# jy0205/Pyramid-Flow

Hardware: NVIDIA H100
Metric: dit_step_latent_tokens_per_sec (higher is better)
Workload: dtype bf16

## Files before the change

### pyramid_flow_b200/csrc/pf_attn.cu

```cuda
#include <algorithm>
#include <vector>

#include "../../include/pf_b200.h"
#include "pf_common.cuh"

namespace pf {

constexpr int ATT_BM = 128;
constexpr int ATT_BN = 128;
constexpr int ATT_HD = 64;
constexpr int ATT_STAGES = 2;
constexpr int ATT_THREADS = 384;
constexpr int ATT_TILE_BYTES = ATT_BN * ATT_HD * 2;
constexpr int ATT_SMEM_BYTES = (1 + 2 * ATT_STAGES) * ATT_TILE_BYTES + 1024;

struct AttnArgs {
  __nv_bfloat16* out;
  long long ldo;
  int batch, heads, seq, q_tiles;
  float scale_log2;
  const int* seg;
  const int* time;
  const int* sched;
  int sched_stride;
  __nv_bfloat16* peer_out[PF_MAX_PEERS];
  int peer_count, peer_chunk_rows, peer_col_begin;
};

__global__ void __launch_bounds__(ATT_THREADS, 1)
attn_fwd_kernel(const __grid_constant__ CUtensorMap tm_q, const __grid_constant__ CUtensorMap tm_k,
                const __grid_constant__ CUtensorMap tm_v, const AttnArgs a) {
  extern __shared__ uint8_t smem_raw[];
  uint8_t* smem = reinterpret_cast<uint8_t*>((reinterpret_cast<uintptr_t>(smem_raw) + 1023) & ~uintptr_t(1023));
  uint8_t* smem_q = smem;
  uint8_t* smem_k = smem + ATT_TILE_BYTES;
  uint8_t* smem_v = smem_k + ATT_STAGES * ATT_TILE_BYTES;

  __shared__ __align__(8) uint64_t bar_q;
  __shared__ __align__(8) uint64_t k_full[ATT_STAGES], k_empty[ATT_STAGES], v_full[ATT_STAGES], v_empty[ATT_STAGES];

  const int warp = threadIdx.x >> 5;
  const int lane = threadIdx.x & 31;
  const int wgroup = warp >> 2;
  const int qt = a.q_tiles - 1 - static_cast<int>(blockIdx.x);
  const int h = blockIdx.y;
  const int b = blockIdx.z;
  const int bh = b * a.heads + h;
  const int* sched = a.sched + (static_cast<size_t>(b) * a.q_tiles + qt) * a.sched_stride;
  const int n_kv = sched[0];

  if (threadIdx.x == 0) {
    tma_prefetch_desc(&tm_q);
    tma_prefetch_desc(&tm_k);
    tma_prefetch_desc(&tm_v);
    mbar_init(&bar_q, 1);
    for (int i = 0; i < ATT_STAGES; ++i) {
      mbar_init(&k_full[i], 1);
      mbar_init(&k_empty[i], 8);
      mbar_init(&v_full[i], 1);
      mbar_init(&v_empty[i], 8);
    }
    fence_barrier_init();
  }
  __syncthreads();

  if (wgroup == 0) {
    setmaxnreg_dec<40>();
    if (warp == 0 && elect_one()) {
      mbar_arrive_expect_tx(&bar_q, ATT_TILE_BYTES);
      tma_load_3d(smem_q, &tm_q, &bar_q, 0, qt * ATT_BM, bh);
      int st = 0;
      uint32_t ph = 0;
      for (int j = 0; j < n_kv; ++j) {
        const int kt = sched[1 + j] >> 1;
        mbar_wait(&k_empty[st], ph ^ 1);
        mbar_arrive_expect_tx(&k_full[st], ATT_TILE_BYTES);
        tma_load_3d(smem_k + st * ATT_TILE_BYTES, &tm_k, &k_full[st], 0, kt * ATT_BN, bh);
        mbar_wait(&v_empty[st], ph ^ 1);
        mbar_arrive_expect_tx(&v_full[st], ATT_TILE_BYTES);
        tma_load_3d(smem_v + st * ATT_TILE_BYTES, &tm_v, &v_full[st], 0, kt * ATT_BN, bh);
        if (++st == ATT_STAGES) {
          st = 0;
          ph ^= 1;
        }
      }
    }
    return;
  }

  setmaxnreg_inc<232>();
  const int wg = wgroup - 1;
  const int g4 = lane >> 2, t4 = lane & 3;
  const int row0 = wg * 64 + (warp & 3) * 16 + g4;
  const float c = a.scale_log2;
  const int* sg = a.seg + static_cast<size_t>(b) * a.seq;
  const int* tm = a.time + static_cast<size_t>(b) * a.seq;
  int seg_q[2], time_q[2];
#pragma unroll
  for (int r = 0; r < 2; ++r) {
    const int qpos = qt * ATT_BM + row0 + 8 * r;
    const bool q_valid = qpos < a.seq;
    seg_q[r] = q_valid ? sg[qpos] : -0x7fffffff;
    time_q[r] = q_valid ? tm[qpos] : -0x7fffffff;
  }
  float m_run[2] = {-INFINITY, -INFINITY};
  float l_run[2] = {0.f, 0.f};
  float o[32];
#pragma unroll
  for (int i = 0; i < 32; ++i) o[i] = 0.f;

  mbar_wait(&bar_q, 0);
  const uint64_t dq = make_smem_desc_kmajor_sw128(smem_u32(smem_q) + wg * (64 * 128));
  int st = 0;
  uint32_t ph = 0;
  for (int j = 0; j < n_kv; ++j) {
    const int entry = sched[1 + j];
    const int kt = entry >> 1;
    const bool masked = (entry & 1) != 0;

    float s[64];
    mbar_wait(&k_full[st], ph);
    {
      const uint64_t dk = make_smem_desc_kmajor_sw128(smem_u32(smem_k + st * ATT_TILE_BYTES));
      wgmma_fence();
#pragma unroll
      for (int kk = 0; kk < ATT_HD / 16; ++kk) wgmma_ss_n128(s, dq + 2 * kk, dk + 2 * kk, kk != 0 ? 1u : 0u);
      wgmma_commit();
      wgmma_wait<0>();
      wgmma_reg_fence(s);
    }
    if (lane == 0) mbar_arrive(&k_empty[st]);

    if (masked) {
#pragma unroll
      for (int i = 0; i < 16; ++i) {
#pragma unroll
        for (int e = 0; e < 2; ++e) {
          const int kv = kt * ATT_BN + 8 * i + 2 * t4 + e;
          int sk = 0x7fffffff, tk = 0x7fffffff;
          if (kv < a.seq) {
            sk = __ldg(sg + kv);
            tk = __ldg(tm + kv);
          }
          if (!(sk == seg_q[0] && tk <= time_q[0])) s[4 * i + e] = -INFINITY;
          if (!(sk == seg_q[1] && tk <= time_q[1])) s[4 * i + 2 + e] = -INFINITY;
        }
      }
    }

    float alpha[2];
#pragma unroll
    for (int r = 0; r < 2; ++r) {
      float mx = -INFINITY;
#pragma unroll
      for (int i = 0; i < 16; ++i) mx = fmaxf(mx, fmaxf(s[4 * i + 2 * r], s[4 * i + 2 * r + 1]));
      mx = fmaxf(mx, __shfl_xor_sync(0xffffffffu, mx, 1));
      mx = fmaxf(mx, __shfl_xor_sync(0xffffffffu, mx, 2));
      const float m_new = fmaxf(m_run[r], mx);
      alpha[r] = (m_new == -INFINITY) ? 1.f : ex2_approx_f((m_run[r] - m_new) * c);
      m_run[r] = m_new;
      const float m_ref = (m_new == -INFINITY) ? 0.f : m_new * c;
      float sum = 0.f;
#pragma unroll
      for (int i = 0; i < 16; ++i) {
        const float p0 = ex2_approx_f(fmaf(s[4 * i + 2 * r], c, -m_ref));
        const float p1 = ex2_approx_f(fmaf(s[4 * i + 2 * r + 1], c, -m_ref));
        s[4 * i + 2 * r] = p0;
        s[4 * i + 2 * r + 1] = p1;
        sum += p0 + p1;
      }
      l_run[r] = l_run[r] * alpha[r] + sum;
    }
#pragma unroll
    for (int i = 0; i < 8; ++i) {
      o[4 * i + 0] *= alpha[0];
      o[4 * i + 1] *= alpha[0];
      o[4 * i + 2] *= alpha[1];
      o[4 * i + 3] *= alpha[1];
    }

    mbar_wait(&v_full[st], ph);
    {
      const uint32_t sv = smem_u32(smem_v + st * ATT_TILE_BYTES);
      uint32_t pa[ATT_BN / 16][4];
#pragma unroll
      for (int kk = 0; kk < ATT_BN / 16; ++kk) {
        pa[kk][0] = pack_bf16x2(s[8 * kk + 0], s[8 * kk + 1]);
        pa[kk][1] = pack_bf16x2(s[8 * kk + 2], s[8 * kk + 3]);
        pa[kk][2] = pack_bf16x2(s[8 * kk + 4], s[8 * kk + 5]);
        pa[kk][3] = pack_bf16x2(s[8 * kk + 6], s[8 * kk + 7]);
      }
      wgmma_reg_fence(o);
      wgmma_fence();
#pragma unroll
      for (int kk = 0; kk < ATT_BN / 16; ++kk) {
        const uint64_t dv = make_smem_desc(sv + kk * 2048, ATT_BN * 128, 1024);
        wgmma_rs_n64_tb(o, pa[kk], dv);
      }
      wgmma_commit();
      wgmma_wait<0>();
      wgmma_reg_fence(o);
    }
    if (lane == 0) mbar_arrive(&v_empty[st]);
    if (++st == ATT_STAGES) {
      st = 0;
      ph ^= 1;
    }
  }

#pragma unroll
  for (int r = 0; r < 2; ++r) {
    float l = l_run[r];
    l += __shfl_xor_sync(0xffffffffu, l, 1);
    l += __shfl_xor_sync(0xffffffffu, l, 2);
    const float inv = (l > 0.f) ? 1.f / l : 0.f;
    const int qpos = qt * ATT_BM + row0 + 8 * r;
    if (qpos >= a.seq) continue;
    __nv_bfloat16* dst;
    if (a.peer_count > 1) {
      const int pr = qpos / a.peer_chunk_rows;
      dst = a.peer_out[pr] + static_cast<size_t>(qpos - pr * a.peer_chunk_rows) * a.ldo + a.peer_col_begin + h * ATT_HD;
    } else {
      dst = a.out + (static_cast<size_t>(b) * a.seq + qpos) * a.ldo + h * ATT_HD;
    }
#pragma unroll
    for (int i = 0; i < 8; ++i)
      *reinterpret_cast<uint32_t*>(dst + 8 * i + 2 * t4) = pack_bf16x2(o[4 * i + 2 * r] * inv, o[4 * i + 2 * r + 1] * inv);
  }
}

int warmup_attn() {
  return ensure_dyn_smem(reinterpret_cast<const void*>(attn_fwd_kernel), ATT_SMEM_BYTES, "attn_fwd_kernel");
}

}

extern "C" int pf_attn_build_schedule(const int32_t* seg, const int32_t* time, int32_t batch, int32_t seq,
                                      int32_t* out, int64_t* allowed_pairs) {
  using namespace pf;
  PF_REQUIRE(batch > 0 && seq > 0, "pf_attn_build_schedule: bad shape");
  const int tiles = (seq + 127) / 128;
  const int stride = 1 + tiles;
  if (out == nullptr) return stride;
  PF_REQUIRE(seg && time, "pf_attn_build_schedule: null ids");
  for (int b = 0; b < batch; ++b) {
    const int32_t* sg = seg + static_cast<size_t>(b) * seq;
    const int32_t* tm = time + static_cast<size_t>(b) * seq;
    std::vector<int32_t> tmin(tiles), tmax(tiles), smin(tiles), smax(tiles);
    for (int t = 0; t < tiles; ++t) {
      const int lo = t * 128, hi = std::min(seq, lo + 128);
      int32_t a = tm[lo], bq = tm[lo], c = sg[lo], d = sg[lo];
      for (int i = lo; i < hi; ++i) {
        a = std::min(a, tm[i]);
        bq = std::max(bq, tm[i]);
        c = std::min(c, sg[i]);
        d = std::max(d, sg[i]);
      }
      tmin[t] = a; tmax[t] = bq; smin[t] = c; smax[t] = d;
    }
    int64_t pairs = 0;
    for (int qt = 0; qt < tiles; ++qt) {
      int32_t* row = out + (static_cast<size_t>(b) * tiles + qt) * stride;
      int cnt = 0;
      const int qlo = qt * 128, qhi = std::min(seq, qlo + 128);
      for (int kt = 0; kt < tiles; ++kt) {
        const int klo = kt * 128, khi = std::min(seq, klo + 128);
        if (tmax[qt] < tmin[kt]) continue;
        if (smax[qt] < smin[kt] || smax[kt] < smin[qt]) continue;
        const bool uniform = (smin[qt] == smax[qt]) && (smin[kt] == smax[kt]) && (smin[qt] == smin[kt]);
        const bool full = uniform && (tmin[qt] >= tmax[kt]) && (khi - klo == 128);
        int64_t n_allowed = 0;
        if (full) {
          n_allowed = static_cast<int64_t>(qhi - qlo) * (khi - klo);
        } else {
          for (int i = qlo; i < qhi; ++i)
            for (int j = klo; j < khi; ++j) n_allowed += (sg[i] == sg[j] && tm[i] >= tm[j]) ? 1 : 0;
          if (n_allowed == 0) continue;
        }
        pairs += n_allowed;
        row[1 + cnt] = (kt << 1) | (full ? 0 : 1);
        ++cnt;
      }
      row[0] = cnt;
      for (int i = 1 + cnt; i < stride; ++i) row[i] = 0;
    }
    if (allowed_pairs) allowed_pairs[b] = pairs;
  }
  return stride;
}

extern "C" int pf_attn_fwd_masked(const pf_attn_desc* d, void* stream_) {
  using namespace pf;
  cudaStream_t stream = static_cast<cudaStream_t>(stream_);
  PF_REQUIRE(d && d->q && d->k && d->v && (d->out || d->peer_count > 1) && d->seg && d->time && d->tile_sched, "pf_attn_fwd_masked: null pointer");
  PF_REQUIRE(d->head_dim == ATT_HD, "pf_attn_fwd_masked: head_dim %d unsupported (64 only)", d->head_dim);
  PF_REQUIRE(d->batch > 0 && d->heads > 0 && d->seq > 0, "pf_attn_fwd_masked: bad shape");
  const int q_tiles = (d->seq + ATT_BM - 1) / ATT_BM;
  PF_REQUIRE(d->sched_stride >= 1 + q_tiles, "pf_attn_fwd_masked: schedule stride %d too small", d->sched_stride);
  PF_REQUIRE(d->q_row_begin >= 0 && d->q_row_begin % ATT_BM == 0 && d->q_row_begin < d->seq,
             "pf_attn_fwd_masked: q_row_begin %d must be a multiple of %d inside the sequence", d->q_row_begin, ATT_BM);
  PF_REQUIRE(d->ldo % 8 == 0 && (reinterpret_cast<uintptr_t>(d->out) & 15) == 0, "pf_attn_fwd_masked: out must be 16-byte aligned");
  PF_REQUIRE(d->variant == 0x10 || d->variant == 0x20 || (d->variant >= 0 && d->variant <= 3), "pf_attn_fwd_masked: bad variant 0x%x", d->variant);
  if (d->variant == 0x20)
    PF_REQUIRE(d->group_sched != nullptr && d->group_mask_index != nullptr && d->group_mask_bits != nullptr,
               "pf_attn_fwd_masked: variant 0x%x needs group_sched, group_mask_index and group_mask_bits", d->variant);
  if (d->variant == 0x10)
    PF_REQUIRE(d->pair_sched != nullptr && d->pair_mask_index != nullptr && d->pair_mask_bits != nullptr,
               "pf_attn_fwd_masked: variant 0x%x needs pair_sched, pair_mask_index and pair_mask_bits", d->variant);
  if (d->peer_count > 1) {
    PF_REQUIRE(d->batch == 1 && d->peer_count <= PF_MAX_PEERS && d->peer_chunk_rows > 0 &&
                   static_cast<long long>(d->peer_chunk_rows) * d->peer_count >= d->seq && d->peer_col_begin % 8 == 0,
               "pf_attn_fwd_masked: bad peer layout (batch %d, count %d, chunk rows %d, seq %d)", d->batch, d->peer_count,
               d->peer_chunk_rows, d->seq);
    for (int i = 0; i < d->peer_count; ++i) PF_REQUIRE(d->peer_out[i] != nullptr, "pf_attn_fwd_masked: peer_out[%d] is null", i);
  }
  CUtensorMap tm[3];
  const void* ptrs[3] = {d->q, d->k, d->v};
  for (int i = 0; i < 3; ++i) {
    const uint64_t dims[3] = {ATT_HD, static_cast<uint64_t>(d->seq), static_cast<uint64_t>(d->batch) * d->heads};
    const uint64_t strides[2] = {ATT_HD * 2, static_cast<uint64_t>(d->seq) * ATT_HD * 2};
    const uint32_t box[3] = {ATT_HD, ATT_BN, 1};
    int rc = encode_tensor_map(&tm[i], CU_TENSOR_MAP_DATA_TYPE_BFLOAT16, 3, ptrs[i], dims, strides, box,
                               CU_TENSOR_MAP_SWIZZLE_128B);
    if (rc) return rc;
  }
  AttnArgs a{};
  a.out = static_cast<__nv_bfloat16*>(d->out);
  a.ldo = d->ldo;
  a.batch = d->batch;
  a.heads = d->heads;
  a.seq = d->seq;
  a.q_tiles = q_tiles;
  a.scale_log2 = d->scale * 1.4426950408889634f;
  a.seg = d->seg;
  a.time = d->time;
  a.sched = d->tile_sched;
  a.sched_stride = d->sched_stride;
  a.peer_count = d->peer_count;
  a.peer_chunk_rows = d->peer_chunk_rows;
  a.peer_col_begin = d->peer_col_begin;
  for (int i = 0; i < PF_MAX_PEERS; ++i) a.peer_out[i] = static_cast<__nv_bfloat16*>(d->peer_out[i]);

  if (int rc = warmup_attn()) return rc;
  dim3 grid(q_tiles - d->q_row_begin / ATT_BM, d->heads, d->batch);
  attn_fwd_kernel<<<grid, ATT_THREADS, ATT_SMEM_BYTES, stream>>>(tm[0], tm[1], tm[2], a);
  return check_launch("pf_attn_fwd_masked");
}
```

### pyramid_flow_b200/csrc/pf_common.cuh

```cuda
#pragma once

#include <cuda.h>
#include <cuda_bf16.h>
#include <cuda_runtime.h>
#include <stdint.h>

namespace pf {

void set_error(const char* fmt, ...);
int  check_launch(const char* what);

#define PF_REQUIRE(cond, ...)                  \
  do {                                         \
    if (!(cond)) {                             \
      ::pf::set_error(__VA_ARGS__);            \
      return -1;                               \
    }                                          \
  } while (0)

int encode_tensor_map(CUtensorMap* map, CUtensorMapDataType dtype, uint32_t rank, const void* base,
                      const uint64_t* dims, const uint64_t* strides_bytes , const uint32_t* box,
                      CUtensorMapSwizzle swizzle,
                      const uint32_t* elem_strides = nullptr );

int num_sms();
int get_option(int key);
int ensure_dyn_smem(const void* kernel, int bytes, const char* what);

__device__ __forceinline__ uint32_t smem_u32(const void* p) {
  return static_cast<uint32_t>(__cvta_generic_to_shared(p));
}

__device__ __forceinline__ bool elect_one() {
  uint32_t pred = 0;
  asm volatile(
      "{\n\t"
      ".reg .b32 %%rx;\n\t"
      ".reg .pred %%px;\n\t"
      "elect.sync %%rx|%%px, 0xffffffff;\n\t"
      "selp.b32 %0, 1, 0, %%px;\n\t"
      "}\n"
      : "=r"(pred));
  return pred != 0;
}

__device__ __forceinline__ void mbar_init(uint64_t* bar, uint32_t count) {
  asm volatile("mbarrier.init.shared::cta.b64 [%0], %1;" ::"r"(smem_u32(bar)), "r"(count) : "memory");
}
__device__ __forceinline__ void fence_barrier_init() {
  asm volatile("fence.mbarrier_init.release.cluster;" ::: "memory");
}
__device__ __forceinline__ void mbar_arrive_expect_tx(uint64_t* bar, uint32_t bytes) {
  asm volatile("mbarrier.arrive.expect_tx.shared::cta.b64 _, [%0], %1;" ::"r"(smem_u32(bar)), "r"(bytes)
               : "memory");
}
__device__ __forceinline__ void mbar_arrive(uint64_t* bar) {
  asm volatile("mbarrier.arrive.shared::cta.b64 _, [%0];" ::"r"(smem_u32(bar)) : "memory");
}
__device__ __forceinline__ bool mbar_try_wait(uint64_t* bar, uint32_t parity) {
  uint32_t ok;
  asm volatile(
      "{\n\t"
      ".reg .pred p;\n\t"
      "mbarrier.try_wait.parity.shared::cta.b64 p, [%1], %2, %3;\n\t"
      "selp.b32 %0, 1, 0, p;\n\t"
      "}\n"
      : "=r"(ok)
      : "r"(smem_u32(bar)), "r"(parity), "r"(0x989680u)
      : "memory");
  return ok != 0;
}
__device__ __forceinline__ bool mbar_test(uint64_t* bar, uint32_t parity) {
  uint32_t ok;
  asm volatile(
      "{\n\t"
      ".reg .pred p;\n\t"
      "mbarrier.test_wait.parity.shared::cta.b64 p, [%1], %2;\n\t"
      "selp.b32 %0, 1, 0, p;\n\t"
      "}\n"
      : "=r"(ok)
      : "r"(smem_u32(bar)), "r"(parity)
      : "memory");
  return ok != 0;
}
__device__ __forceinline__ void mbar_wait(uint64_t* bar, uint32_t parity) {
  while (!mbar_try_wait(bar, parity)) {
  }
}

__device__ __forceinline__ void tma_prefetch_desc(const CUtensorMap* m) {
  asm volatile("prefetch.tensormap [%0];" ::"l"(reinterpret_cast<uint64_t>(m)) : "memory");
}
__device__ __forceinline__ void tma_load_2d(void* smem_dst, const CUtensorMap* m, uint64_t* bar, int c0, int c1) {
  asm volatile(
      "cp.async.bulk.tensor.2d.shared::cluster.global.mbarrier::complete_tx::bytes [%0], [%1, {%3, %4}], [%2];"
      ::"r"(smem_u32(smem_dst)), "l"(reinterpret_cast<uint64_t>(m)), "r"(smem_u32(bar)), "r"(c0), "r"(c1)
      : "memory");
}
__device__ __forceinline__ void tma_load_3d(void* smem_dst, const CUtensorMap* m, uint64_t* bar, int c0, int c1,
                                            int c2) {
  asm volatile(
      "cp.async.bulk.tensor.3d.shared::cluster.global.mbarrier::complete_tx::bytes [%0], [%1, {%3, %4, %5}], [%2];"
      ::"r"(smem_u32(smem_dst)), "l"(reinterpret_cast<uint64_t>(m)), "r"(smem_u32(bar)), "r"(c0), "r"(c1), "r"(c2)
      : "memory");
}
__device__ __forceinline__ void tma_load_4d(void* smem_dst, const CUtensorMap* m, uint64_t* bar, int c0, int c1,
                                            int c2, int c3) {
  asm volatile(
      "cp.async.bulk.tensor.4d.shared::cluster.global.mbarrier::complete_tx::bytes [%0], [%1, {%3, %4, %5, %6}], "
      "[%2];" ::"r"(smem_u32(smem_dst)),
      "l"(reinterpret_cast<uint64_t>(m)), "r"(smem_u32(bar)), "r"(c0), "r"(c1), "r"(c2), "r"(c3)
      : "memory");
}
__device__ __forceinline__ void tma_load_5d(void* smem_dst, const CUtensorMap* m, uint64_t* bar, int c0, int c1,
                                            int c2, int c3, int c4) {
  asm volatile(
      "cp.async.bulk.tensor.5d.shared::cluster.global.mbarrier::complete_tx::bytes [%0], [%1, {%3, %4, %5, %6, "
      "%7}], [%2];" ::"r"(smem_u32(smem_dst)),
      "l"(reinterpret_cast<uint64_t>(m)), "r"(smem_u32(bar)), "r"(c0), "r"(c1), "r"(c2), "r"(c3), "r"(c4)
      : "memory");
}
__device__ __forceinline__ void fence_proxy_async_smem() {
  asm volatile("fence.proxy.async.shared::cta;" ::: "memory");
}
__device__ __forceinline__ void tma_load_2d_multicast(void* smem_dst, const CUtensorMap* m, uint64_t* bar, int c0, int c1,
                                                      uint16_t cta_mask) {
  asm volatile(
      "cp.async.bulk.tensor.2d.shared::cluster.global.mbarrier::complete_tx::bytes.multicast::cluster [%0], [%1, {%3, %4}], "
      "[%2], %5;" ::"r"(smem_u32(smem_dst)),
      "l"(reinterpret_cast<uint64_t>(m)), "r"(smem_u32(bar)), "r"(c0), "r"(c1), "h"(cta_mask)
      : "memory");
}

__device__ __forceinline__ uint32_t cluster_ctarank() {
  uint32_t r;
  asm volatile("mov.u32 %0, %%cluster_ctarank;" : "=r"(r));
  return r;
}
__device__ __forceinline__ void mbar_arrive_cluster(uint64_t* bar, uint32_t cta) {
  asm volatile(
      "{\n\t"
      ".reg .b32 ra;\n\t"
      "mapa.shared::cluster.u32 ra, %0, %1;\n\t"
      "mbarrier.arrive.shared::cluster.b64 _, [ra];\n\t"
      "}\n" ::"r"(smem_u32(bar)), "r"(cta)
      : "memory");
}
__device__ __forceinline__ void cluster_arrive() { asm volatile("barrier.cluster.arrive.release.aligned;" ::: "memory"); }
__device__ __forceinline__ void cluster_wait() { asm volatile("barrier.cluster.wait.acquire.aligned;" ::: "memory"); }

__device__ __forceinline__ void wgmma_fence() { asm volatile("wgmma.fence.sync.aligned;" ::: "memory"); }
__device__ __forceinline__ void wgmma_commit() { asm volatile("wgmma.commit_group.sync.aligned;" ::: "memory"); }
template <int N>
__device__ __forceinline__ void wgmma_wait() {
  asm volatile("wgmma.wait_group.sync.aligned %0;" ::"n"(N) : "memory");
}
template <int N>
__device__ __forceinline__ void wgmma_reg_fence(float (&d)[N]) {
#pragma unroll
  for (int i = 0; i < N; ++i) asm volatile("" : "+f"(d[i])::"memory");
}
template <int REGS>
__device__ __forceinline__ void setmaxnreg_inc() {
  asm volatile("setmaxnreg.inc.sync.aligned.u32 %0;" ::"n"(REGS));
}
template <int REGS>
__device__ __forceinline__ void setmaxnreg_dec() {
  asm volatile("setmaxnreg.dec.sync.aligned.u32 %0;" ::"n"(REGS));
}
__device__ __forceinline__ void named_bar_sync(int id, int threads) {
  asm volatile("bar.sync %0, %1;" ::"r"(id), "r"(threads) : "memory");
}

__device__ __forceinline__ void wgmma_ss_n128(float (&d)[64], uint64_t desc_a, uint64_t desc_b, uint32_t accumulate) {
  asm volatile(
      "{\n\t"
      ".reg .pred p;\n\t"
      "setp.ne.b32 p, %66, 0;\n\t"
      "wgmma.mma_async.sync.aligned.m64n128k16.f32.bf16.bf16 "
      "{%0, %1, %2, %3, %4, %5, %6, %7, %8, %9, %10, %11, %12, %13, %14, %15, %16, %17, %18, %19, %20, %21, %22, %23, %24, %25, %26, %27, %28, %29, %30, %31, %32, %33, %34, %35, %36, %37, %38, %39, %40, %41, %42, %43, %44, %45, %46, %47, %48, %49, %50, %51, %52, %53, %54, %55, %56, %57, %58, %59, %60, %61, %62, %63}, %64, %65, p, 1, 1, 0, 0;\n\t"
      "}\n"
      : "+f"(d[0]), "+f"(d[1]), "+f"(d[2]), "+f"(d[3]), "+f"(d[4]), "+f"(d[5]), "+f"(d[6]), "+f"(d[7]), "+f"(d[8]), "+f"(d[9]), "+f"(d[10]), "+f"(d[11]), "+f"(d[12]), "+f"(d[13]), "+f"(d[14]), "+f"(d[15]), "+f"(d[16]), "+f"(d[17]), "+f"(d[18]), "+f"(d[19]), "+f"(d[20]), "+f"(d[21]), "+f"(d[22]), "+f"(d[23]), "+f"(d[24]), "+f"(d[25]), "+f"(d[26]), "+f"(d[27]), "+f"(d[28]), "+f"(d[29]), "+f"(d[30]), "+f"(d[31]), "+f"(d[32]), "+f"(d[33]), "+f"(d[34]), "+f"(d[35]), "+f"(d[36]), "+f"(d[37]), "+f"(d[38]), "+f"(d[39]), "+f"(d[40]), "+f"(d[41]), "+f"(d[42]), "+f"(d[43]), "+f"(d[44]), "+f"(d[45]), "+f"(d[46]), "+f"(d[47]), "+f"(d[48]), "+f"(d[49]), "+f"(d[50]), "+f"(d[51]), "+f"(d[52]), "+f"(d[53]), "+f"(d[54]), "+f"(d[55]), "+f"(d[56]), "+f"(d[57]), "+f"(d[58]), "+f"(d[59]), "+f"(d[60]), "+f"(d[61]), "+f"(d[62]), "+f"(d[63])
      : "l"(desc_a), "l"(desc_b), "r"(accumulate)
      : "memory");
}
__device__ __forceinline__ void wgmma_ss_n64(float (&d)[32], uint64_t desc_a, uint64_t desc_b, uint32_t accumulate) {
  asm volatile(
      "{\n\t"
      ".reg .pred p;\n\t"
      "setp.ne.b32 p, %34, 0;\n\t"
      "wgmma.mma_async.sync.aligned.m64n64k16.f32.bf16.bf16 "
      "{%0, %1, %2, %3, %4, %5, %6, %7, %8, %9, %10, %11, %12, %13, %14, %15, %16, %17, %18, %19, %20, %21, %22, %23, %24, %25, %26, %27, %28, %29, %30, %31}, %32, %33, p, 1, 1, 0, 0;\n\t"
      "}\n"
      : "+f"(d[0]), "+f"(d[1]), "+f"(d[2]), "+f"(d[3]), "+f"(d[4]), "+f"(d[5]), "+f"(d[6]), "+f"(d[7]), "+f"(d[8]), "+f"(d[9]), "+f"(d[10]), "+f"(d[11]), "+f"(d[12]), "+f"(d[13]), "+f"(d[14]), "+f"(d[15]), "+f"(d[16]), "+f"(d[17]), "+f"(d[18]), "+f"(d[19]), "+f"(d[20]), "+f"(d[21]), "+f"(d[22]), "+f"(d[23]), "+f"(d[24]), "+f"(d[25]), "+f"(d[26]), "+f"(d[27]), "+f"(d[28]), "+f"(d[29]), "+f"(d[30]), "+f"(d[31])
      : "l"(desc_a), "l"(desc_b), "r"(accumulate)
      : "memory");
}
__device__ __forceinline__ void wgmma_rs_n64_tb(float (&d)[32], const uint32_t (&a)[4], uint64_t desc_b) {
  asm volatile(
      "{\n\t"
      ".reg .pred p;\n\t"
      "setp.ne.b32 p, 1, 0;\n\t"
      "wgmma.mma_async.sync.aligned.m64n64k16.f32.bf16.bf16 "
      "{%0, %1, %2, %3, %4, %5, %6, %7, %8, %9, %10, %11, %12, %13, %14, %15, %16, %17, %18, %19, %20, %21, %22, %23, %24, %25, %26, %27, %28, %29, %30, %31}, {%32, %33, %34, %35}, %36, p, 1, 1, 1;\n\t"
      "}\n"
      : "+f"(d[0]), "+f"(d[1]), "+f"(d[2]), "+f"(d[3]), "+f"(d[4]), "+f"(d[5]), "+f"(d[6]), "+f"(d[7]), "+f"(d[8]), "+f"(d[9]), "+f"(d[10]), "+f"(d[11]), "+f"(d[12]), "+f"(d[13]), "+f"(d[14]), "+f"(d[15]), "+f"(d[16]), "+f"(d[17]), "+f"(d[18]), "+f"(d[19]), "+f"(d[20]), "+f"(d[21]), "+f"(d[22]), "+f"(d[23]), "+f"(d[24]), "+f"(d[25]), "+f"(d[26]), "+f"(d[27]), "+f"(d[28]), "+f"(d[29]), "+f"(d[30]), "+f"(d[31])
      : "r"(a[0]), "r"(a[1]), "r"(a[2]), "r"(a[3]), "l"(desc_b)
      : "memory");
}
template <int BN>
__device__ __forceinline__ void wgmma_ss(float (&d)[BN / 2], uint64_t desc_a, uint64_t desc_b, uint32_t accumulate) {
  static_assert(BN == 128 || BN == 64, "wgmma_ss: tile widths 128 and 64 are instantiated");
  if constexpr (BN == 128) wgmma_ss_n128(d, desc_a, desc_b, accumulate);
  else wgmma_ss_n64(d, desc_a, desc_b, accumulate);
}

__device__ __forceinline__ uint64_t make_smem_desc(uint32_t saddr, uint32_t lbo_bytes, uint32_t sbo_bytes) {
  uint64_t d = 0;
  d |= static_cast<uint64_t>((saddr & 0x3FFFFu) >> 4);
  d |= static_cast<uint64_t>((lbo_bytes >> 4) & 0x3FFFu) << 16;
  d |= static_cast<uint64_t>((sbo_bytes >> 4) & 0x3FFFu) << 32;
  d |= static_cast<uint64_t>(1) << 62;
  return d;
}
__device__ __forceinline__ uint64_t make_smem_desc_kmajor_sw128(uint32_t saddr) {
  return make_smem_desc(saddr, 16, 1024);
}

constexpr int PIPE_THREADS = 384;
constexpr int PIPE_CONSUMER_WARPS = 8;
constexpr int PIPE_BM = 128;
constexpr int PIPE_BK = 64;
template <int BN>
struct PipeCfg {
  static constexpr int A_BYTES = PIPE_BM * PIPE_BK * 2;
  static constexpr int B_BYTES = BN * PIPE_BK * 2;
  static constexpr int STAGE_BYTES = A_BYTES + B_BYTES;
  static constexpr int STAGES = (BN >= 128) ? 4 : 6;
  static constexpr int ACC_PITCH = BN + 8;
  static constexpr int ACC_BYTES = PIPE_BM * ACC_PITCH * 4;
  static constexpr int SMEM_BYTES = STAGES * STAGE_BYTES + ACC_BYTES + 1024;
};

template <int BN>
__device__ __forceinline__ void pipe_consume_tile(float (&acc)[BN / 2], uint8_t* smem, uint64_t* full_bar, uint64_t* empty_bar,
                                                  int num_kb, int wg, int& stage, uint32_t& phase) {
  using Cfg = PipeCfg<BN>;
  const int lane = threadIdx.x & 31;
  int prev = -1;
  for (int kb = 0; kb < num_kb; ++kb) {
    mbar_wait(&full_bar[stage], phase);
    const uint32_t sa = smem_u32(smem + stage * Cfg::STAGE_BYTES);
    const uint64_t da = make_smem_desc_kmajor_sw128(sa + wg * (64 * 128));
    const uint64_t db = make_smem_desc_kmajor_sw128(sa + Cfg::A_BYTES);
    wgmma_reg_fence(acc);
    wgmma_fence();
#pragma unroll
    for (int kk = 0; kk < PIPE_BK / 16; ++kk) wgmma_ss<BN>(acc, da + 2 * kk, db + 2 * kk, (kb | kk) != 0 ? 1u : 0u);
    wgmma_commit();
    wgmma_wait<1>();
    if (prev >= 0 && lane == 0) mbar_arrive(&empty_bar[prev]);
    prev = stage;
    if (++stage == Cfg::STAGES) {
      stage = 0;
      phase ^= 1;
    }
  }
  wgmma_wait<0>();
  wgmma_reg_fence(acc);
  if (prev >= 0 && lane == 0) mbar_arrive(&empty_bar[prev]);
}

template <int BN>
__device__ __forceinline__ void pipe_stage_acc(const float (&acc)[BN / 2], float* acc_tile, int wg) {
  const int w = (threadIdx.x >> 5) & 3, lane = threadIdx.x & 31;
  float* r0 = acc_tile + (wg * 64 + w * 16 + (lane >> 2)) * PipeCfg<BN>::ACC_PITCH + 2 * (lane & 3);
  float* r1 = r0 + 8 * PipeCfg<BN>::ACC_PITCH;
#pragma unroll
  for (int i = 0; i < BN / 8; ++i) {
    *reinterpret_cast<float2*>(r0 + 8 * i) = make_float2(acc[4 * i + 0], acc[4 * i + 1]);
    *reinterpret_cast<float2*>(r1 + 8 * i) = make_float2(acc[4 * i + 2], acc[4 * i + 3]);
  }
}

__device__ __forceinline__ uint32_t pack_bf16x2(float lo, float hi) {
  __nv_bfloat162 v = __floats2bfloat162_rn(lo, hi);
  return *reinterpret_cast<uint32_t*>(&v);
}
__device__ __forceinline__ float rcp_approx_f(float x) {
  float y;
  asm("rcp.approx.ftz.f32 %0, %1;" : "=f"(y) : "f"(x));
  return y;
}
__device__ __forceinline__ float ex2_approx_f(float x) {
  float y;
  asm("ex2.approx.ftz.f32 %0, %1;" : "=f"(y) : "f"(x));
  return y;
}
__device__ __forceinline__ float gelu_tanh_f(float x) {
  const float c0 = -2.0f * 0.7978845608028654f * 1.4426950408889634f;
  const float c1 = c0 * 0.044715f;
  const float x2 = x * x;
  const float nu = x * fmaf(x2, c1, c0);
  return x * rcp_approx_f(1.0f + ex2_approx_f(nu));
}
__device__ __forceinline__ float silu_f(float x) {
  return x * rcp_approx_f(1.0f + ex2_approx_f(-1.4426950408889634f * x));
}

}
```

Before: 126,300.

## Overlap QK and PV wgmma across iterations with ping-pong warpgroup scheduling

New measurement: 128,700, median of 6. +1.9%, better.

```diff
diff --git a/pyramid_flow_b200/csrc/pf_attn.cu b/pyramid_flow_b200/csrc/pf_attn.cu
--- a/pyramid_flow_b200/csrc/pf_attn.cu
+++ b/pyramid_flow_b200/csrc/pf_attn.cu
@@ -26,6 +26,81 @@
   __nv_bfloat16* peer_out[PF_MAX_PEERS];
   int peer_count, peer_chunk_rows, peer_col_begin;
 };
+
+__device__ __forceinline__ void issue_qk(float (&s)[64], uint64_t dq, const uint8_t* k_tile) {
+  const uint64_t dk = make_smem_desc_kmajor_sw128(smem_u32(k_tile));
+  wgmma_reg_fence(s);
+  wgmma_fence();
+#pragma unroll
+  for (int kk = 0; kk < ATT_HD / 16; ++kk) wgmma_ss_n128(s, dq + 2 * kk, dk + 2 * kk, kk != 0 ? 1u : 0u);
+  wgmma_commit();
+  wgmma_reg_fence(s);
+}
+
+__device__ __forceinline__ void issue_pv(float (&o)[32], uint32_t (&pa)[ATT_BN / 16][4], const uint8_t* v_tile) {
+  const uint32_t sv = smem_u32(v_tile);
+  wgmma_reg_fence(o);
+  wgmma_reg_fence(pa);
+  wgmma_fence();
+#pragma unroll
+  for (int kk = 0; kk < ATT_BN / 16; ++kk) wgmma_rs_n64_tb(o, pa[kk], make_smem_desc(sv + kk * 2048, ATT_BN * 128, 1024));
+  wgmma_commit();
+  wgmma_reg_fence(o);
+  wgmma_reg_fence(pa);
+}
+
+__device__ __forceinline__ void mask_tile(float (&s)[64], int kv0, int seq, const int* sg, const int* tm, const int (&seg_q)[2],
+                                          const int (&time_q)[2]) {
+#pragma unroll
+  for (int i = 0; i < 16; ++i) {
+#pragma unroll
+    for (int e = 0; e < 2; ++e) {
+      const int kv = kv0 + 8 * i + e;
+      int sk = 0x7fffffff, tk = 0x7fffffff;
+      if (kv < seq) {
+        sk = __ldg(sg + kv);
+        tk = __ldg(tm + kv);
+      }
+      if (!(sk == seg_q[0] && tk <= time_q[0])) s[4 * i + e] = -INFINITY;
+      if (!(sk == seg_q[1] && tk <= time_q[1])) s[4 * i + 2 + e] = -INFINITY;
+    }
+  }
+}
+
+__device__ __forceinline__ void online_softmax(float (&s)[64], float (&m_run)[2], float (&l_run)[2], float (&alpha)[2], float c) {
+#pragma unroll
+  for (int r = 0; r < 2; ++r) {
+    float mx = -INFINITY;
+#pragma unroll
+    for (int i = 0; i < 16; ++i) mx = fmaxf(mx, fmaxf(s[4 * i + 2 * r], s[4 * i + 2 * r + 1]));
+    mx = fmaxf(mx, __shfl_xor_sync(0xffffffffu, mx, 1));
+    mx = fmaxf(mx, __shfl_xor_sync(0xffffffffu, mx, 2));
+    const float m_new = fmaxf(m_run[r], mx);
+    alpha[r] = (m_new == -INFINITY) ? 1.f : ex2_approx_f((m_run[r] - m_new) * c);
+    m_run[r] = m_new;
+    const float m_ref = (m_new == -INFINITY) ? 0.f : m_new * c;
+    float sum = 0.f;
+#pragma unroll
+    for (int i = 0; i < 16; ++i) {
+      const float p0 = ex2_approx_f(fmaf(s[4 * i + 2 * r], c, -m_ref));
+      const float p1 = ex2_approx_f(fmaf(s[4 * i + 2 * r + 1], c, -m_ref));
+      s[4 * i + 2 * r] = p0;
+      s[4 * i + 2 * r + 1] = p1;
+      sum += p0 + p1;
+    }
+    l_run[r] = l_run[r] * alpha[r] + sum;
+  }
+}
+
+__device__ __forceinline__ void pack_p(uint32_t (&pa)[ATT_BN / 16][4], const float (&s)[64]) {
+#pragma unroll
+  for (int kk = 0; kk < ATT_BN / 16; ++kk) {
+    pa[kk][0] = pack_bf16x2(s[8 * kk + 0], s[8 * kk + 1]);
+    pa[kk][1] = pack_bf16x2(s[8 * kk + 2], s[8 * kk + 3]);
+    pa[kk][2] = pack_bf16x2(s[8 * kk + 4], s[8 * kk + 5]);
+    pa[kk][3] = pack_bf16x2(s[8 * kk + 6], s[8 * kk + 7]);
+  }
+}
 
 __global__ void __launch_bounds__(ATT_THREADS, 1)
 attn_fwd_kernel(const __grid_constant__ CUtensorMap tm_q, const __grid_constant__ CUtensorMap tm_k,
@@ -110,102 +185,69 @@
   for (int i = 0; i < 32; ++i) o[i] = 0.f;
 
   mbar_wait(&bar_q, 0);
-  const uint64_t dq = make_smem_desc_kmajor_sw128(smem_u32(smem_q) + wg * (64 * 128));
-  int st = 0;
-  uint32_t ph = 0;
-  for (int j = 0; j < n_kv; ++j) {
-    const int entry = sched[1 + j];
-    const int kt = entry >> 1;
-    const bool masked = (entry & 1) != 0;
-
+  if (n_kv > 0) {
+    const int bar_mine = 1 + wg, bar_other = 2 - wg;
+    if (wg == 1) named_bar_arrive(bar_other, 256);
+
+    const uint64_t dq = make_smem_desc_kmajor_sw128(smem_u32(smem_q) + wg * (64 * 128));
     float s[64];
-    mbar_wait(&k_full[st], ph);
-    {
-      const uint64_t dk = make_smem_desc_kmajor_sw128(smem_u32(smem_k + st * ATT_TILE_BYTES));
-      wgmma_fence();
-#pragma unroll
-      for (int kk = 0; kk < ATT_HD / 16; ++kk) wgmma_ss_n128(s, dq + 2 * kk, dk + 2 * kk, kk != 0 ? 1u : 0u);
-      wgmma_commit();
-      wgmma_wait<0>();
+    uint32_t pa[ATT_BN / 16][4];
+    float alpha[2];
+
+    int st = 0;
+    uint32_t ph = 0;
+    int entry = sched[1];
+    named_bar_sync(bar_mine, 256);
+    mbar_wait(&k_full[0], 0);
+    issue_qk(s, dq, smem_k);
+    named_bar_arrive(bar_other, 256);
+    wgmma_wait<0>();
+    wgmma_reg_fence(s);
+    if (lane == 0) mbar_arrive(&k_empty[0]);
+    if (entry & 1) mask_tile(s, (entry >> 1) * ATT_BN + 2 * t4, a.seq, sg, tm, seg_q, time_q);
+    online_softmax(s, m_run, l_run, alpha, c);
+    pack_p(pa, s);
+
+    for (int j = 1; j < n_kv; ++j) {
+      const int pst = st;
+      const uint32_t pph = ph;
+      if (++st == ATT_STAGES) {
+        st = 0;
+        ph ^= 1;
+      }
+      entry = sched[1 + j];
+      named_bar_sync(bar_mine, 256);
+      mbar_wait(&k_full[st], ph);
+      issue_qk(s, dq, smem_k + st * ATT_TILE_BYTES);
+      mbar_wait(&v_full[pst], pph);
+      issue_pv(o, pa, smem_v + pst * ATT_TILE_BYTES);
+      named_bar_arrive(bar_other, 256);
+      wgmma_wait<1>();
       wgmma_reg_fence(s);
-    }
-    if (lane == 0) mbar_arrive(&k_empty[st]);
-
-    if (masked) {
-#pragma unroll
-      for (int i = 0; i < 16; ++i) {
-#pragma unroll
-        for (int e = 0; e < 2; ++e) {
-          const int kv = kt * ATT_BN + 8 * i + 2 * t4 + e;
-          int sk = 0x7fffffff, tk = 0x7fffffff;
-          if (kv < a.seq) {
-            sk = __ldg(sg + kv);
-            tk = __ldg(tm + kv);
-          }
-          if (!(sk == seg_q[0] && tk <= time_q[0])) s[4 * i + e] = -INFINITY;
-          if (!(sk == seg_q[1] && tk <= time_q[1])) s[4 * i + 2 + e] = -INFINITY;
-        }
-      }
-    }
-
-    float alpha[2];
-#pragma unroll
-    for (int r = 0; r < 2; ++r) {
-      float mx = -INFINITY;
-#pragma unroll
-      for (int i = 0; i < 16; ++i) mx = fmaxf(mx, fmaxf(s[4 * i + 2 * r], s[4 * i + 2 * r + 1]));
-      mx = fmaxf(mx, __shfl_xor_sync(0xffffffffu, mx, 1));
-      mx = fmaxf(mx, __shfl_xor_sync(0xffffffffu, mx, 2));
-      const float m_new = fmaxf(m_run[r], mx);
-      alpha[r] = (m_new == -INFINITY) ? 1.f : ex2_approx_f((m_run[r] - m_new) * c);
-      m_run[r] = m_new;
-      const float m_ref = (m_new == -INFINITY) ? 0.f : m_new * c;
-      float sum = 0.f;
-#pragma unroll
-      for (int i = 0; i < 16; ++i) {
-        const float p0 = ex2_approx_f(fmaf(s[4 * i + 2 * r], c, -m_ref));
-        const float p1 = ex2_approx_f(fmaf(s[4 * i + 2 * r + 1], c, -m_ref));
-        s[4 * i + 2 * r] = p0;
-        s[4 * i + 2 * r + 1] = p1;
-        sum += p0 + p1;
-      }
-      l_run[r] = l_run[r] * alpha[r] + sum;
-    }
-#pragma unroll
-    for (int i = 0; i < 8; ++i) {
-      o[4 * i + 0] *= alpha[0];
-      o[4 * i + 1] *= alpha[0];
-      o[4 * i + 2] *= alpha[1];
-      o[4 * i + 3] *= alpha[1];
-    }
-
-    mbar_wait(&v_full[st], ph);
-    {
-      const uint32_t sv = smem_u32(smem_v + st * ATT_TILE_BYTES);
-      uint32_t pa[ATT_BN / 16][4];
-#pragma unroll
-      for (int kk = 0; kk < ATT_BN / 16; ++kk) {
-        pa[kk][0] = pack_bf16x2(s[8 * kk + 0], s[8 * kk + 1]);
-        pa[kk][1] = pack_bf16x2(s[8 * kk + 2], s[8 * kk + 3]);
-        pa[kk][2] = pack_bf16x2(s[8 * kk + 4], s[8 * kk + 5]);
-        pa[kk][3] = pack_bf16x2(s[8 * kk + 6], s[8 * kk + 7]);
-      }
-      wgmma_reg_fence(o);
-      wgmma_fence();
-#pragma unroll
-      for (int kk = 0; kk < ATT_BN / 16; ++kk) {
-        const uint64_t dv = make_smem_desc(sv + kk * 2048, ATT_BN * 128, 1024);
-        wgmma_rs_n64_tb(o, pa[kk], dv);
-      }
-      wgmma_commit();
+      if (lane == 0) mbar_arrive(&k_empty[st]);
+      if (entry & 1) mask_tile(s, (entry >> 1) * ATT_BN + 2 * t4, a.seq, sg, tm, seg_q, time_q);
+      online_softmax(s, m_run, l_run, alpha, c);
       wgmma_wait<0>();
       wgmma_reg_fence(o);
-    }
+      wgmma_reg_fence(pa);
+      if (lane == 0) mbar_arrive(&v_empty[pst]);
+#pragma unroll
+      for (int i = 0; i < 8; ++i) {
+        o[4 * i + 0] *= alpha[0];
+        o[4 * i + 1] *= alpha[0];
+        o[4 * i + 2] *= alpha[1];
+        o[4 * i + 3] *= alpha[1];
+      }
+      pack_p(pa, s);
+    }
+
+    named_bar_sync(bar_mine, 256);
+    mbar_wait(&v_full[st], ph);
+    issue_pv(o, pa, smem_v + st * ATT_TILE_BYTES);
+    if (wg == 0) named_bar_arrive(bar_other, 256);
+    wgmma_wait<0>();
+    wgmma_reg_fence(o);
     if (lane == 0) mbar_arrive(&v_empty[st]);
-    if (++st == ATT_STAGES) {
-      st = 0;
-      ph ^= 1;
-    }
   }
 
 #pragma unroll
diff --git a/pyramid_flow_b200/csrc/pf_common.cuh b/pyramid_flow_b200/csrc/pf_common.cuh
--- a/pyramid_flow_b200/csrc/pf_common.cuh
+++ b/pyramid_flow_b200/csrc/pf_common.cuh
@@ -160,6 +160,13 @@
 #pragma unroll
   for (int i = 0; i < N; ++i) asm volatile("" : "+f"(d[i])::"memory");
 }
+template <int M, int N>
+__device__ __forceinline__ void wgmma_reg_fence(uint32_t (&a)[M][N]) {
+#pragma unroll
+  for (int i = 0; i < M; ++i)
+#pragma unroll
+    for (int k = 0; k < N; ++k) asm volatile("" : "+r"(a[i][k])::"memory");
+}
 template <int REGS>
 __device__ __forceinline__ void setmaxnreg_inc() {
   asm volatile("setmaxnreg.inc.sync.aligned.u32 %0;" ::"n"(REGS));
@@ -170,6 +177,9 @@
 }
 __device__ __forceinline__ void named_bar_sync(int id, int threads) {
   asm volatile("bar.sync %0, %1;" ::"r"(id), "r"(threads) : "memory");
+}
+__device__ __forceinline__ void named_bar_arrive(int id, int threads) {
+  asm volatile("bar.arrive %0, %1;" ::"r"(id), "r"(threads) : "memory");
 }
 
 __device__ __forceinline__ void wgmma_ss_n128(float (&d)[64], uint64_t desc_a, uint64_t desc_b, uint32_t accumulate) {
```
